# compbioproj-cdna-to-genome-map-align/gmap-2024

Measured on AMD Instinct MI355X. Metric: aligned cDNA reads/sec (2 kb, GRCh38) at 1/2/4/8 MI355X; DP HBM GB/s vs peak, higher is better.
Workload: dtype int32

## Files before the change

### gmap-2024_amd/csrc/oi_kernel.hip

```cpp
#include <cstdlib>

#include "dp_device.h"

namespace gmapdp {

constexpr int kOiK = 8;

#ifdef GMAPDP_OI_TIMING
__device__ unsigned long long g_oi_marks[2][16];
__device__ unsigned int g_oi_wave[3][16384];
#define OI_MARK(k)                                                 \
  do {                                                             \
    if (threadIdx.x == 0) {                                        \
      atomicAdd(&g_oi_marks[0][k], (unsigned long long)wall_clock64()); \
      atomicAdd(&g_oi_marks[1][k], 1ull);                          \
    }                                                              \
  } while (0)
#else
#define OI_MARK(k) \
  do {             \
  } while (0)
#endif
constexpr int kOiWords = 65536 / 32;

// ... 342 lines not shown
      c_mk = ((uint64_t)(uint32_t)__builtin_amdgcn_readlane((int)(mk >> 32), 63) << 32) |
             (uint32_t)__builtin_amdgcn_readlane((int)(uint32_t)mk, 63);
      c_key = KT::readlane(key_r, 63);
    }
  }
#pragma unroll
  for (int off = 32; off >= 1; off >>= 1) {
    const int om = __shfl_xor(bm, off, 64);
    const uint64_t ok = __shfl_xor(bkey, off, 64);
    const int oe = __shfl_xor(be, off, 64);
    if (om > bm || (om == bm && ok < bkey)) {
      bm = om;
      bkey = ok;
      be = oe;
    }
  }
  const int M = max(bm, 0);
  __threadfence_block();
  if (ngood == 0 && M > 0) {
    if (lane == 0) grec[0] = make_int4(-1, be, M, (int)(uint32_t)bkey);
    ngood = 1;
  }
  __threadfence_block();
  for (int g = lane; g < ngood; g += 64) {
    const int4 r = grec[g];
    const uint32_t di = (uint32_t)r.w;
    const int eb = r.y, bn = r.z;
    const uint32_t qreach = r.x >= 0 ? KT::q(S[r.x], cum, nq) : 0u;
    gkey[g] = ((uint64_t)qreach << 32) | di;
    grec[g] = make_int4(di >= (uint32_t)qlen ? (int)(di - (uint32_t)qlen) : (int)((uint32_t)qlen - di),
                        (int)KT::q(S[eb - bn], cum, nq), (int)KT::q(S[eb], cum, nq), bn + 1);
  }
  __threadfence_block();
  if (ngood > gcap) ngood = -1;
  for (int g = lane; g < ngood; g += 64) {
    const uint64_t k = gkey[g];
    int rank = 0;
    for (int h = 0; h < ngood; h++) rank += gkey[h] < k ? 1 : 0;
    reinterpret_cast<int4*>(good)[rank] = grec[g];
  }
  maxn_out = M;
  return ngood;
}

constexpr int kOimSlots = 1024;
__device__ __forceinline__ uint32_t oim_slot(uint32_t di) { return (di * 2654435761u) >> 22; }

template <typename KT, bool kSlots>
__device__ bool oi_mappings_sorted(int lane, int qlen, int nq, int E, uint32_t maxdiag, uint32_t chrinit,
                                   int lookback, int suffn, const int32_t* __restrict__ npq,
                                   const int32_t* __restrict__ mpq, const int* __restrict__ cum,
                                   const uint32_t* __restrict__ table_all, uint64_t* __restrict__ pool,
                                   unsigned long long base, uint32_t* hist,
                                   int* evq, int32_t* __restrict__ good, int gcap, int& ngood_out, int& maxn_out,
                                   uint32_t* slots = nullptr) {
  OI_MARK(9);
  if (base == ~0ull) return false;
  using K = typename KT::K;
  K* evA = reinterpret_cast<K*>(pool + base);
  K* evB = evA + E;
  int4* grec = reinterpret_cast<int4*>(pool + base + 2 * (size_t)E);
  const OiDigits D = oi_digits(maxdiag);
  const uint32_t need = (uint32_t)suffn + 1u;
  bool filtered = kSlots && E < 65536;
  if (filtered) {
    for (int i = lane; i < kOimSlots / 2; i += 64) slots[i] = 0u;
    oi_wave_sync();
    oi_for_events<KT>(lane, qlen, nq, chrinit, npq, mpq, cum, table_all, evq, [&](int, bool v, uint32_t di, K) {
      if (v) {
        const uint32_t h = oim_slot(di);
        atomicAdd(&slots[h >> 1], 1u << (16 * (h & 1)));
      }
    });
    oi_wave_sync();
  }
  for (;;) {
    for (int i = lane; i < kOiHist; i += 64) hist[i] = 0u;
    oi_wave_sync();
    int C = 0;
    oi_for_events<KT>(lane, qlen, nq, chrinit, npq, mpq, cum, table_all, evq,
                      [&](int, bool v, uint32_t di, K key) {
                        bool c = v;
                        if (filtered) {
                          const uint32_t h = oim_slot(di);
                          c = v && ((slots[h >> 1] >> (16 * (h & 1))) & 0xFFFFu) >= need;
                        }
                        const uint64_t cm = ballot(c);
                        if (c) evA[C + lanes_below(cm, lane)] = key;
                        oi_hist_add(lane, c, di, D, hist);
                        C += __popcll(cm);
                      });
    __threadfence_block();
    oi_wave_sync();
    OI_MARK(5);
    const K* S = oi_radix<KT>(lane, evA, evB, C, D, hist);
    OI_MARK(6);
    uint64_t* gkey = sizeof(K) == 8 ? reinterpret_cast<uint64_t*>(S == evA ? evB : evA) : pool + base + E;
    int maxn = 0;
    const int ngood = oi_sweep<KT>(lane, S, C, qlen, nq, lookback, suffn, cum, grec, gkey, good, gcap, maxn);
    if (filtered && ngood != -1 && (ngood == 0 || maxn < suffn)) {
      filtered = false;
      continue;
    }
    ngood_out = ngood;
    maxn_out = maxn;
    return true;
  }
}

template <typename CT>
__device__ __forceinline__ void count_inc(CT* cnt, int u) {
  if constexpr (sizeof(CT) == 4) {
    atomicAdd(reinterpret_cast<uint32_t*>(cnt) + u, 1u);
  } else {
    atomicAdd(reinterpret_cast<uint32_t*>(cnt) + (u >> 1), 1u << (16 * (u & 1)));
  }
}

__device__ void oi_report_overflow(const DevOligoProblem& P, int tid, int nthreads, int qlen, int32_t* npq,
                                   int32_t* mpq, gmapdp_oligo_result* results, unsigned char* poolslot) {
  for (int i = tid; i < qlen; i += nthreads) {
    npq[i] = 0;
    mpq[i] = -1;
  }
  if (tid == 0) {
    gmapdp_oligo_result res;
    res.totalpositions = 0;
    res.maxnconsecutive = 0;
    res.oned_matrix_p = -1;
    res.ndiagonals = 0;
    res.table_offset = P.table_offset;
    res.diag_offset = P.diag_offset;
    results[P.index] = res;
    *reinterpret_cast<unsigned long long*>(poolslot) = ~0ull;
  }
}

constexpr int kOiWaves = 2;
#ifdef GMAPDP_OI_STAGE
constexpr bool kOiStage = true;
#else
constexpr bool kOiStage = false;
#endif

#define OI_PASS_ARGS                                                                                          \
  const DevOligoProblem *__restrict__ probs, const uint32_t *__restrict__ blocks, const char *__restrict__ quc_all, \
      unsigned char *__restrict__ scratch, gmapdp_oligo_result *__restrict__ results,                             \
      int32_t *__restrict__ npos_out, int32_t *__restrict__ map_out, uint32_t *__restrict__ table_all,            \
      unsigned long long *__restrict__ pool_counter, unsigned long long pool_cap, int32_t *__restrict__ nhits_out
template <typename CT>
__device__ __forceinline__ void oi_pass(OI_PASS_ARGS) {
  extern __shared__ __attribute__((aligned(16))) unsigned char smem[];
  __shared__ int nh_wave[kOiWaves];
  const int tid = threadIdx.x, lane = tid & 63;
  const int wave = __builtin_amdgcn_readfirstlane(tid >> 6);
  const DevOligoProblem P = probs[blockIdx.x];
  uint32_t* bitmap = reinterpret_cast<uint32_t*>(smem);
  uint16_t* wrank = reinterpret_cast<uint16_t*>(smem + 4 * kOiWords);
  CT* cnt = reinterpret_cast<CT*>(smem + 6 * kOiWords);
  CT* offs = cnt + P.umax;
  const char* quc = quc_all + P.qoff;
  const int qlen = P.querylength;
  OI_MARK(0);
#ifdef GMAPDP_OI_TIMING
  const unsigned long long oi_t0 = wall_clock64();
#endif
  const int nq = qlen - kOiK + 1;

  for (int w = tid; w < kOiWords; w += 64 * kOiWaves) bitmap[w] = 0u;
  __syncthreads();
  int32_t* npq = npos_out + P.qoff;
  int32_t* mpq = map_out + P.qoff;
  for (int sb = 4 * 64 * wave; sb < qlen; sb += 4 * 64 * kOiWaves) {
    int ch[5];
#pragma unroll
    for (int r = 0; r < 5; r++) {
      const int i = sb + 64 * r + lane;
      ch[r] = i < qlen ? nt_code(quc[i]) : -1;
    }
#pragma unroll
    for (int r = 0; r < 4; r++) {
      const int i = sb + 64 * r + lane;
      uint32_t m = 0;
      bool ok = i < nq;
#pragma unroll
      for (int j = 0; j < kOiK; j++) {
        const int src = (lane + j) & 63;
        const int a = __shfl(ch[r], src, 64), b = __shfl(ch[r + 1], src, 64);
        const int cj = lane + j < 64 ? a : b;
        ok = ok && cj >= 0;
        m = (m << 2) | ((uint32_t)cj & 3u);
      }
      if (i < qlen) {
        mpq[i] = ok ? (int)m : -1;
        npq[i] = 0;
      }
      if (ok) atomicOr(&bitmap[m >> 5], 1u << (m & 31));
    }
  }
  __syncthreads();
  int run = 0;
  for (int base = 0; base < kOiWords; base += 64) {
    const int c = __popc(bitmap[base + lane]);
    const int incl = wave_scan_add(lane, c);
    if (wave == 0) wrank[base + lane] = (uint16_t)(run + incl - c);
    run += __builtin_amdgcn_readlane(incl, 63);
  }
  const int U = run;
  OI_MARK(1);
  unsigned char* base_s = scratch + P.scratch_offset;
  const ScratchOi so = scratch_oi(qlen, P.chrend > P.chrstart ? P.chrend - P.chrstart : 0);
  if (U > P.umax) {
    oi_report_overflow(P, tid, 64 * kOiWaves, qlen, npq, mpq, results, base_s + so.poolbase);
    return;
  }
  for (int u = tid; u < U; u += 64 * kOiWaves) cnt[u] = 0;
  __syncthreads();

  const uint64_t left = (uint64_t)P.chroffset + P.chrstart;
  uint64_t lpl = (uint64_t)P.chroffset + P.chrend + (P.plusp ? 0 : 1);
  lpl = lpl < (uint64_t)kOiK ? 0 : lpl - kOiK;
  const uint64_t npos = lpl > left ? lpl - left + 1 : 0;
  uint2* hitlist = reinterpret_cast<uint2*>(base_s + so.hits);
  uint32_t* hitlist32 = reinterpret_cast<uint32_t*>(base_s + so.hits);
  const bool compact = npos <= (1ull << 18);
  int nhits = 0;
  if (npos > 0) {
    const uint64_t hlo0 = left >> 4, hhi0 = lpl >> 4;
    const uint64_t nsteps = (hhi0 - hlo0) / 64 + 1, half = (nsteps + 1) / 2;
    const uint64_t hlo = hlo0 + (wave ? 64 * half : 0);
    const uint64_t hhi = wave ? hhi0 : (hlo0 + 64 * half - 1 < hhi0 ? hlo0 + 64 * half - 1 : hhi0);
    constexpr int kOiAhead = 4;
    uint32_t pw0[kOiAhead], pw1[kOiAhead];
#pragma unroll
    for (int a = 0; a < kOiAhead; a++) {
      const uint64_t hh = hlo + 64 * a + lane;
      pw0[a] = hh <= hhi ? half_word(blocks, hh) : 0u;
      pw1[a] = hh <= hhi ? half_word(blocks, hh + 1) : 0u;
    }
    auto step = [&](uint64_t hb, uint64_t v) {
      const uint64_t h = hb + lane;
      uint64_t vv;
      if (P.plusp) {
        vv = ((v >> 2) & 0x3333333333333333ull) | ((v & 0x3333333333333333ull) << 2);
        vv = ((vv >> 4) & 0x0F0F0F0F0F0F0F0Full) | ((vv & 0x0F0F0F0F0F0F0F0Full) << 4);
        vv = __builtin_bswap64(vv);
      } else {
        vv = ~v;
      }
      auto oligo_at = [&](int j) -> uint32_t {
        return (uint32_t)(vv >> (P.plusp ? 2 * (24 - j) : 2 * j)) & 0xFFFFu;
      };
      uint32_t vmask = 0;
      if (h <= hhi) {
        const uint64_t p0 = 16 * h;
        const int jlo = left > p0 ? (int)(left - p0) : 0;
        const int jhi = lpl < p0 + 15 ? (int)(lpl - p0) : 15;
        if (jlo <= jhi) vmask = (0xFFFFu >> (15 - jhi)) & (0xFFFFu << jlo);
      }
      uint32_t hm = 0;
#pragma unroll
      for (int j = 0; j < 16; j++) {
        const uint32_t m = oligo_at(j);
        hm |= ((bitmap[m >> 5] >> (m & 31)) & 1u) << j;
      }
      hm &= vmask;
      const int c = __popc(hm);
      const int incl = wave_scan_add(lane, c);
      int o = nhits + incl - c;
      for (uint32_t r = hm; r; r &= r - 1) {
        const int j = __ffs(r) - 1;
        const uint32_t m = oligo_at(j);
        bool in;
        const int id = oligo_id(bitmap, wrank, m, in);
        count_inc(cnt, id);
        if ((uint32_t)o < P.hit_cap) {
          const uint32_t at = wave ? P.hit_cap - 1 - (uint32_t)o : (uint32_t)o;
          const uint32_t k = (uint32_t)(16 * h + j - left);
          if (compact) hitlist32[at] = (k << 14) | (uint32_t)id;
          else hitlist[at] = make_uint2(k, (uint32_t)id);
        }
        o++;
      }
      nhits += __builtin_amdgcn_readlane(incl, 63);
    };
    for (uint64_t hb0 = hlo; hlo <= hhi && hb0 <= hhi; hb0 += 64 * kOiAhead) {
#pragma unroll
      for (int a = 0; a < kOiAhead; a++) {
        const uint64_t hb = hb0 + 64 * a;
        if (hb > hhi) break;
        const uint64_t v = (uint64_t)pw0[a] | ((uint64_t)pw1[a] << 32);
        const uint64_t hh = hb + 64 * kOiAhead + lane;
        pw0[a] = hh <= hhi ? half_word(blocks, hh) : 0u;
        pw1[a] = hh <= hhi ? half_word(blocks, hh + 1) : 0u;
        step(hb, v);
      }
    }
  }
  if (lane == 0) nh_wave[wave] = nhits;
  __syncthreads();
  const int n0 = nh_wave[0], n1 = nh_wave[1];
  nhits = n0 + n1;
  if (nhits_out && tid == 0) nhits_out[P.index] = nhits;
  __shared__ uint32_t tot_s;
  if (wave == 0) {
    uint32_t tot = 0;
    for (int base = 0; base < U; base += 64) {
      const int u = base + lane;
      const uint32_t c = u < U ? ((uint32_t)cnt[u] & 255u) : 0u;
      const uint32_t incl = (uint32_t)wave_scan_add(lane, (int)c);
      if (u < U) {
        offs[u] = (CT)(tot + incl - c);
        cnt[u] = (CT)c;
      }
      tot += (uint32_t)__builtin_amdgcn_readlane((int)incl, 63);
    }
    if (lane == 0) tot_s = tot;
  }
  for (int i = tid; i < nq; i += 64 * kOiWaves) {
    const int m = mpq[i];
    if (m >= 0) {
      bool in;
      mpq[i] = oligo_id(bitmap, wrank, (uint32_t)m, in);
    }
  }
  __syncthreads();
  const uint32_t tot = tot_s;
  OI_MARK(2);
  if ((uint32_t)nhits > P.hit_cap || tot > P.table_cap || (sizeof(CT) == 2 && nhits > 65535)) {
    oi_report_overflow(P, tid, 64 * kOiWaves, qlen, npq, mpq, results, base_s + so.poolbase);
    return;
  }

  uint32_t* table = table_all + P.table_offset;
  uint32_t* slotarr = hitlist32 + P.hit_cap;
  const uint32_t chrpos0 = P.plusp ? P.chrstart : (P.chrhigh - P.chroffset) - P.chrend;
  const int idbits = U > 1 ? 32 - __clz(U - 1) : 1;
  __threadfence_block();
  for (int c = 0; wave == 0 && c < nhits; c += 64) {
    const int sl = c + lane;
    int id = -1;
    uint32_t k = 0, at = 0;
    if (sl < nhits) {
      const int a = P.plusp ? nhits - 1 - sl : sl;
      at = a < n0 ? (uint32_t)a : P.hit_cap - 1 - (uint32_t)(a - n0);
      if (compact) {
        const uint32_t e = hitlist32[at];
        k = e >> 14;
        id = (int)(e & 0x3FFFu);
      } else {
        const uint2 hv = hitlist[at];
        k = hv.x;
        id = (int)hv.y;
      }
    }
    const uint64_t hits = ballot(id >= 0);
    uint64_t eq = hits;
    for (int b = 0; b < idbits; b++) {
      const uint64_t m = ballot((id >> b) & 1);
      eq &= ((id >> b) & 1) ? m : ~m;
    }
    if (id >= 0) {
      const int rank = lanes_below(eq, lane);
      const int same = __popcll(eq);
      const int r0 = (int)cnt[id];
      const uint32_t slot = (uint32_t)offs[id] + (uint32_t)(r0 - rank - 1);
      if (kOiStage && compact)
        slotarr[at] = r0 - rank > 0 ? slot : 0xFFFFFFFFu;
      else if (r0 - rank > 0)
        table[slot] = chrpos0 + (P.plusp ? k : (uint32_t)(npos - 1) - k);
      if (rank == 0) cnt[id] = (CT)max(r0 - same, 0);
    }
  }
  __threadfence_block();
  __syncthreads();
  if (kOiStage && compact) {
    uint32_t* stage = reinterpret_cast<uint32_t*>(smem);
    constexpr uint32_t kStage = 6 * kOiWords / 4;
    for (uint32_t b0 = 0; b0 < tot; b0 += kStage) {
      for (int a = tid; a < nhits; a += 64 * kOiWaves) {
        const uint32_t at = a < n0 ? (uint32_t)a : P.hit_cap - 1 - (uint32_t)(a - n0);
        const uint32_t sd = slotarr[at] - b0;
        if (sd < kStage) {
          const uint32_t k = hitlist32[at] >> 14;
          stage[sd] = chrpos0 + (P.plusp ? k : (uint32_t)(npos - 1) - k);
        }
      }
      __syncthreads();
      const uint32_t nb = min(kStage, tot - b0);
      for (uint32_t j = tid; j < nb; j += 64 * kOiWaves) table[b0 + j] = stage[j];
      __syncthreads();
    }
  }
  OI_MARK(3);
  for (int u = tid; u < U; u += 64 * kOiWaves)
    cnt[u] = (CT)((u + 1 < U ? (uint32_t)offs[u + 1] : tot) - (uint32_t)offs[u]);
  __threadfence_block();
  __syncthreads();
  if (wave) return;

  gmapdp_oligo_result res;
  res.totalpositions = 0;
  res.maxnconsecutive = 0;
  res.oned_matrix_p = 0;
  res.ndiagonals = 0;
  res.table_offset = P.table_offset;
  res.diag_offset = P.diag_offset;
  __threadfence_block();
  int* cum = reinterpret_cast<int*>(base_s);
  int totalpositions = 0, cumrun = 0;
  for (int sb = 0; sb < nq; sb += 4 * 64) {
    int mm[4];
#pragma unroll
    for (int r = 0; r < 4; r++) {
      const int i = sb + 64 * r + lane;
      mm[r] = i < nq ? mpq[i] : -1;
    }
#pragma unroll
    for (int r = 0; r < 4; r++) {
      const int i = sb + 64 * r + lane;
      const int m = mm[r];
      int nh = -1;
      if (i < nq) {
        int mo = -1;
        if (m >= 0) {
          const int u = m;
          nh = (int)cnt[u];
          npq[i] = nh;
          if (nh > 0) mo = (int32_t)(uint32_t)offs[u];
        }
        mpq[i] = mo;
      }
      const int incl = wave_scan_add(lane, nh == 0 ? 1 : 0);
      if (i < nq) cum[i] = cumrun + incl;
      cumrun += __builtin_amdgcn_readlane(incl, 63);
      totalpositions += __builtin_amdgcn_readlane(wave_scan_add(lane, nh > 0 ? nh : 0), 63);
    }
  }
  __threadfence_block();
  res.totalpositions = totalpositions;
  if (lane == 0) {
    results[P.index] = res;
    unsigned long long b = ~0ull;
    if (P.chrend > P.chrstart) {
      const unsigned long long need = 3ull * (unsigned long long)totalpositions;
      b = atomicAdd(pool_counter, need);
      if (b + need > pool_cap) b = ~0ull;
    }
    *reinterpret_cast<unsigned long long*>(base_s + so.poolbase) = b;
  }
  OI_MARK(4);
#ifdef GMAPDP_OI_TIMING
  if (lane == 0 && P.index < 16384) g_oi_wave[0][P.index] = (unsigned int)(wall_clock64() - oi_t0);
#endif
}

__device__ bool oi_mappings_walk(int lane, const DevOligoProblem& P, unsigned char* __restrict__ scratch, int qlen,
                                 int nq, const int32_t* __restrict__ npq, const int32_t* __restrict__ mpq,
                                 const int* __restrict__ cum, const uint32_t* __restrict__ table, uint32_t chrinit,
                                 int diag_lookback, int suffn, int32_t* __restrict__ good, int& ngood_out,
                                 int& maxn_out) {
  if (P.fallback_offset < 0) return false;
  const ScratchOiFb fb = scratch_oi_fb(qlen, P.chrend - P.chrstart);
  unsigned char* initp = scratch + P.fallback_offset + fb.initp;
  OiState* st = reinterpret_cast<OiState*>(scratch + P.fallback_offset + fb.states);
  for (size_t b = 16 * (size_t)lane; b < fb.states - fb.initp; b += 16 * 64)
    *reinterpret_cast<uint4*>(initp + b) = make_uint4(0u, 0u, 0u, 0u);
  __threadfence_block();
  int best = -1;
  int ngood = 0, maxn = 0;
  for (int cb = 0; cb < nq; cb += 64) {
    const int qi = cb + lane;
    int c_nh = 0, c_mo = 0, c_cum = 0;
    uint32_t c_h0 = 0;
    if (qi < nq) {
      c_nh = npq[qi];
      c_mo = mpq[qi];
      c_cum = cum[qi];
      if (c_nh > 0) c_h0 = table[c_mo];
    }
    const int cend = min(64, nq - cb);
    for (int j = 0; j < cend; j++) {
      const int nh = __builtin_amdgcn_readlane(c_nh, j);
      if (nh <= 0) continue;
      const int q = cb + j;
      const int mo = __builtin_amdgcn_readlane(c_mo, j);
      const int cq = __builtin_amdgcn_readlane(c_cum, j);
      const uint32_t h0 = (uint32_t)__builtin_amdgcn_readlane((int)c_h0, j);
      for (int base = 0; base < nh; base += 64) {
        const int h = base + lane;
        int reached = 0, nb = 0;
        uint32_t diagi = 0;
        if (h < nh) {
          diagi = (h == 0 ? h0 : table[mo + h]) + (uint32_t)(qlen - q) - chrinit;
          const unsigned char ini = initp[diagi];
          OiState s = st[diagi];
          if (!ini) {
            initp[diagi] = 1;
            s.querypos = -diag_lookback;
            s.best_n = s.n = s.cstart = s.best_start = s.best_end = 0;
          }
          if (s.querypos < 0) {
            s.n = 0;
            s.cstart = q;
          } else if (q - s.querypos >= diag_lookback + cq - cum[s.querypos]) {
            s.n = 0;
            s.cstart = q;
          } else if (++s.n > s.best_n) {
            s.best_start = s.cstart;
            s.best_end = q;
            s.best_n = s.n;
            reached = (s.best_n == suffn);
            nb = s.best_n;
          }
          s.querypos = q;
          st[diagi] = s;
        }
        const uint64_t rm = ballot(reached);
        if (reached && ngood + lanes_below(rm, lane) < (int)min(P.diag_cap, 0x7fffffffu))
          good[4 * (ngood + lanes_below(rm, lane))] = (int32_t)diagi;
        ngood += __popcll(rm);
        int mx = nb;
#pragma unroll
        for (int off = 32; off >= 1; off >>= 1) mx = max(mx, __shfl_xor(mx, off, 64));
        if (mx > maxn) {
          const int l = __ffsll((long long)ballot(nb == mx)) - 1;
          best = __builtin_amdgcn_readlane((int)diagi, l);
          maxn = mx;
        }
      }
    }
  }
  if (ngood == 0 && maxn > 0) {
    if (lane == 0 && P.diag_cap > 0) good[0] = best;
    ngood = 1;
  }
  __threadfence_block();
  if ((uint32_t)ngood > P.diag_cap) ngood = -1;
  for (int g = lane; g < ngood; g += 64) {
    const int di = good[4 * g];
    const OiState s = st[di];
    good[4 * g + 0] = di >= qlen ? di - qlen : qlen - di;
    good[4 * g + 1] = s.best_start;
    good[4 * g + 2] = s.best_end;
    good[4 * g + 3] = s.best_n + 1;
  }
  ngood_out = ngood;
  maxn_out = maxn;
  return true;
}

template <bool kSlots>
__device__ void oi_mappings_global(int lane, const DevOligoProblem& P, unsigned char* __restrict__ scratch, int qlen,
                                   int nq, int E, const int32_t* __restrict__ npq, const int32_t* __restrict__ mpq,
                                   const int* __restrict__ cum, const uint32_t* __restrict__ table,
                                   uint64_t* __restrict__ pool, unsigned long long pbase, uint32_t* hist, int* evq,
                                   int32_t* __restrict__ good, gmapdp_oligo_result* __restrict__ results,
                                   uint32_t* slots = nullptr) {
  const int diag_lookback = P.minor ? 60 : 120, suffn = P.minor ? 10 : 20;
  const uint32_t chrinit = P.plusp ? P.chrstart : (P.chrhigh - P.chroffset) - P.chrend;
  int ngood = 0, maxn = 0;
  const uint32_t maxdiag = (uint32_t)qlen + (P.chrend - P.chrstart);
  const int gcap = (int)min(P.diag_cap, 0x7fffffffu);
  const bool sorted =
      maxdiag < (1u << 20) - 1 && nq <= 4096
          ? oi_mappings_sorted<OiKeyT32, kSlots>(lane, qlen, nq, E, maxdiag, chrinit, diag_lookback, suffn, npq, mpq, cum,
                                         table, pool, pbase, hist, evq, good, gcap, ngood, maxn, slots)
      : nq < 65536
          ? oi_mappings_sorted<OiKeyQT, kSlots>(lane, qlen, nq, E, maxdiag, chrinit, diag_lookback, suffn, npq, mpq, cum,
                                        table, pool, pbase, hist, evq, good, gcap, ngood, maxn, slots)
          : oi_mappings_sorted<OiKeyQ, kSlots>(lane, qlen, nq, E, maxdiag, chrinit, diag_lookback, suffn, npq, mpq, cum,
                                       table, pool, pbase, hist, evq, good, gcap, ngood, maxn, slots);
  if (!sorted && !oi_mappings_walk(lane, P, scratch, qlen, nq, npq, mpq, cum, table, chrinit, diag_lookback, suffn,
                                   good, ngood, maxn))
    ngood = -1;
  if (lane == 0) {
    results[P.index].maxnconsecutive = ngood < 0 ? 0 : maxn;
    results[P.index].oned_matrix_p = ngood < 0 ? -1 : 1;
    results[P.index].ndiagonals = max(ngood, 0);
  }
}

template <typename CT>
__global__ __launch_bounds__(64 * kOiWaves) void oi_kernel(OI_PASS_ARGS) {
  oi_pass<CT>(probs, blocks, quc_all, scratch, results, npos_out, map_out, table_all, pool_counter, pool_cap,
              nhits_out);
}
template <typename CT>
__global__ __launch_bounds__(64 * kOiWaves) void oi_size_kernel(OI_PASS_ARGS) {
  oi_pass<CT>(probs, blocks, quc_all, scratch, results, npos_out, map_out, table_all, pool_counter, pool_cap,
              nhits_out);
}

#define OI_MAP_ARGS                                                                                           \
  const DevOligoProblem *__restrict__ probs, unsigned char *__restrict__ scratch,                                 \
      gmapdp_oligo_result *__restrict__ results, const int32_t *__restrict__ npos_out,                            \
      const int32_t *__restrict__ map_out, const uint32_t *__restrict__ table_all, int32_t *__restrict__ diag_all, \
      uint64_t *__restrict__ pool
__device__ __forceinline__ void oi_map_pass(OI_MAP_ARGS) {
  __shared__ uint32_t hist[kOiHist];
  __shared__ int evq[3 * 256];
  __shared__ uint32_t slots[kOimSlots / 2];
  const int lane = threadIdx.x;
  const DevOligoProblem P = probs[blockIdx.x];
  if (P.chrend <= P.chrstart) return;
  if (results[P.index].oned_matrix_p < 0) return;
  OI_MARK(8);
#ifdef GMAPDP_OI_TIMING
  const unsigned long long om_t0 = wall_clock64();
#endif
  const int qlen = P.querylength;
  const int nq = qlen - kOiK + 1;
  unsigned char* base_s = scratch + P.scratch_offset;
  const ScratchOi so = scratch_oi(qlen, P.chrend - P.chrstart);
  const int totalpositions = results[P.index].totalpositions;
  oi_mappings_global<true>(lane, P, scratch, qlen, nq, totalpositions, npos_out + P.qoff, map_out + P.qoff,
                     reinterpret_cast<const int*>(base_s), table_all + P.table_offset, pool,
                     *reinterpret_cast<const unsigned long long*>(base_s + so.poolbase), hist, evq,
                     diag_all + 4 * P.diag_offset, results, slots);
  OI_MARK(7);
#ifdef GMAPDP_OI_TIMING
  if (lane == 0 && P.index < 16384) {
    g_oi_wave[1][P.index] = (unsigned int)(wall_clock64() - om_t0);
    g_oi_wave[2][P.index] = (unsigned int)totalpositions;
  }
#endif
}

__global__ __launch_bounds__(64) void oi_map_kernel(OI_MAP_ARGS) {
  oi_map_pass(probs, scratch, results, npos_out, map_out, table_all, diag_all, pool);
}
__global__ __launch_bounds__(64) void oi_size_map_kernel(OI_MAP_ARGS) {
  oi_map_pass(probs, scratch, results, npos_out, map_out, table_all, diag_all, pool);
}


template <typename F>
__device__ __forceinline__ void oi_query_oligos(int lane, const char* __restrict__ quc, int qlen, int nq, int sb,
                                                F&& f) {
  int ch[5];
#pragma unroll
  for (int r = 0; r < 5; r++) {
    const int i = sb + 64 * r + lane;
    ch[r] = i < qlen ? nt_code(quc[i]) : -1;
  }
#pragma unroll
  for (int r = 0; r < 4; r++) {
    const int i = sb + 64 * r + lane;
    uint32_t m = 0;
    bool ok = i < nq;
#pragma unroll
    for (int j = 0; j < kOiK; j++) {
      const int src = (lane + j) & 63;
      const int a = __shfl(ch[r], src, 64), b = __shfl(ch[r + 1], src, 64);
      const int cj = lane + j < 64 ? a : b;
      ok = ok && cj >= 0;
      m = (m << 2) | ((uint32_t)cj & 3u);
    }
    f(i, ok, m);
  }
}

struct OiWindow {
  uint64_t left, lpl, npos;
  bool compact;
};
__device__ __forceinline__ OiWindow oi_window(const DevOligoProblem& P) {
  OiWindow w;
  w.left = (uint64_t)P.chroffset + P.chrstart;
  uint64_t lpl = (uint64_t)P.chroffset + P.chrend + (P.plusp ? 0 : 1);
  w.lpl = lpl < (uint64_t)kOiK ? 0 : lpl - kOiK;
  w.npos = w.lpl > w.left ? w.lpl - w.left + 1 : 0;
  w.compact = w.npos <= (1ull << 18);
  return w;
}

__global__ __launch_bounds__(64 * kOiWaves) void oi_scan_kernel(
    const DevOligoProblem* __restrict__ probs, const uint32_t* __restrict__ blocks, const char* __restrict__ quc_all,
    unsigned char* __restrict__ scratch, int32_t* __restrict__ npos_out, int32_t* __restrict__ map_out) {
  __shared__ uint32_t bitmap[kOiWords];
  __shared__ uint16_t wrank[kOiWords];
  __shared__ int nh_wave[kOiWaves];
  const int tid = threadIdx.x, lane = tid & 63;
  const int wave = __builtin_amdgcn_readfirstlane(tid >> 6);
  const DevOligoProblem P = probs[blockIdx.x];
  const char* quc = quc_all + P.qoff;
  const int qlen = P.querylength;
  const int nq = qlen - kOiK + 1;
  OI_MARK(10);
  for (int w = tid; w < kOiWords; w += 64 * kOiWaves) bitmap[w] = 0u;
  __syncthreads();
  for (int sb = 4 * 64 * wave; sb < qlen; sb += 4 * 64 * kOiWaves)
    oi_query_oligos(lane, quc, qlen, nq, sb, [&](int, bool ok, uint32_t m) {
      if (ok) atomicOr(&bitmap[m >> 5], 1u << (m & 31));
    });
  __syncthreads();
  int run = 0;
  for (int base = 0; base < kOiWords; base += 64) {
    const int c = __popc(bitmap[base + lane]);
    const int incl = wave_scan_add(lane, c);
    if (wave == 0) wrank[base + lane] = (uint16_t)(run + incl - c);
    run += __builtin_amdgcn_readlane(incl, 63);
  }
  const int U = run;
  __syncthreads();
  int32_t* npq = npos_out + P.qoff;
  int32_t* mpq = map_out + P.qoff;
  for (int sb = 4 * 64 * wave; sb < qlen; sb += 4 * 64 * kOiWaves)
    oi_query_oligos(lane, quc, qlen, nq, sb, [&](int i, bool ok, uint32_t m) {
      if (i < qlen) {
        bool in;
        mpq[i] = ok ? oligo_id(bitmap, wrank, m, in) : -1;
        npq[i] = 0;
      }
    });

  const OiWindow W = oi_window(P);
  const uint64_t left = W.left, lpl = W.lpl;
  unsigned char* base_s = scratch + P.scratch_offset;
  const ScratchOi so = scratch_oi(qlen, P.chrend > P.chrstart ? P.chrend - P.chrstart : 0);
  uint32_t* hl32 = reinterpret_cast<uint32_t*>(base_s + so.hits);
  uint2* hl64 = reinterpret_cast<uint2*>(base_s + so.hits);
  int nhits = 0;
  if (W.npos > 0) {
    const uint64_t hlo0 = left >> 4, hhi0 = lpl >> 4;
    const uint64_t nsteps = (hhi0 - hlo0) / 64 + 1, half = (nsteps + 1) / 2;
    const uint64_t hlo = hlo0 + (wave ? 64 * half : 0);
    const uint64_t hhi = wave ? hhi0 : (hlo0 + 64 * half - 1 < hhi0 ? hlo0 + 64 * half - 1 : hhi0);
    constexpr int kOiAhead = 4;
    uint32_t pw0[kOiAhead], pw1[kOiAhead];
#pragma unroll
    for (int a = 0; a < kOiAhead; a++) {
      const uint64_t hh = hlo + 64 * a + lane;
      pw0[a] = hh <= hhi ? half_word(blocks, hh) : 0u;
      pw1[a] = hh <= hhi ? half_word(blocks, hh + 1) : 0u;
    }
    auto step = [&](uint64_t hb, uint64_t v) {
      const uint64_t h = hb + lane;
      uint64_t vv;
      if (P.plusp) {
        vv = ((v >> 2) & 0x3333333333333333ull) | ((v & 0x3333333333333333ull) << 2);
        vv = ((vv >> 4) & 0x0F0F0F0F0F0F0F0Full) | ((vv & 0x0F0F0F0F0F0F0F0Full) << 4);
        vv = __builtin_bswap64(vv);
// ... 462 lines not shown
```

Measured before the change: 347,000.

## Fuse offset scan with per-query mapping pass and software-pipeline hit scatter loads

Merges the per-unique-oligo prefix scan, the oligo_id remapping loop and the final per-query cum/npq pass into a single wave-0 loop over queries. Offsets are assigned on first occurrence using ballot-based duplicate detection and a visited bit in cnt. The hit-scatter loop now prefetches the next batch of hitlist entries into registers before processing the current one. The per-unique recount pass is dropped. This removes two shared-memory passes and a block-wide remap loop, but the work is serialized onto one wave, adds extra ballots per query, and table order now follows first query occurrence.

```diff
diff --git a/gmap-2024_amd/csrc/oi_kernel.hip b/gmap-2024_amd/csrc/oi_kernel.hip
--- a/gmap-2024_amd/csrc/oi_kernel.hip
+++ b/gmap-2024_amd/csrc/oi_kernel.hip
@@ -668,27 +668,66 @@
   const int n0 = nh_wave[0], n1 = nh_wave[1];
   nhits = n0 + n1;
   if (nhits_out && tid == 0) nhits_out[P.index] = nhits;
+  for (int u = tid; u < U; u += 64 * kOiWaves) cnt[u] = (CT)((uint32_t)cnt[u] & 255u);
+  __syncthreads();
   __shared__ uint32_t tot_s;
+  const int idbits = U > 1 ? 32 - __clz(U - 1) : 1;
+  int* cum = reinterpret_cast<int*>(base_s);
+  int totalpositions = 0;
   if (wave == 0) {
     uint32_t tot = 0;
-    for (int base = 0; base < U; base += 64) {
-      const int u = base + lane;
-      const uint32_t c = u < U ? ((uint32_t)cnt[u] & 255u) : 0u;
-      const uint32_t incl = (uint32_t)wave_scan_add(lane, (int)c);
-      if (u < U) {
-        offs[u] = (CT)(tot + incl - c);
-        cnt[u] = (CT)c;
-      }
-      tot += (uint32_t)__builtin_amdgcn_readlane((int)incl, 63);
+    int cumrun = 0;
+    for (int sb = 0; sb < nq; sb += 4 * 64) {
+      int mm[4];
+#pragma unroll
+      for (int r = 0; r < 4; r++) {
+        const int i = sb + 64 * r + lane;
+        mm[r] = i < nq ? mpq[i] : -1;
+      }
+#pragma unroll
+      for (int r = 0; r < 4; r++) {
+        if (sb + 64 * r >= nq) break;
+        const int i = sb + 64 * r + lane;
+        int id = -1;
+        uint32_t cv = 0;
+        if (mm[r] >= 0) {
+          bool in;
+          id = oligo_id(bitmap, wrank, (uint32_t)mm[r], in);
+          cv = (uint32_t)cnt[id];
+        }
+        const bool cand = id >= 0 && (cv >> 8) == 0u;
+        uint64_t eq = ballot(cand);
+        for (int b = 0; b < idbits; b++) {
+          const uint64_t m = ballot((id >> b) & 1);
+          eq &= ((id >> b) & 1) ? m : ~m;
+        }
+        const bool first = cand && lanes_below(eq, lane) == 0;
+        const uint32_t kept = cv & 255u;
+        const uint32_t c = first ? kept : 0u;
+        const uint32_t incl = (uint32_t)wave_scan_add(lane, (int)c);
+        if (first) {
+          offs[id] = (CT)(tot + incl - c);
+          cnt[id] = (CT)(cv | 0x100u);
+        }
+        tot += (uint32_t)__builtin_amdgcn_readlane((int)incl, 63);
+        oi_wave_sync();
+        int nh = -1;
+        if (i < nq) {
+          int mo = -1;
+          if (id >= 0) {
+            nh = (int)kept;
+            npq[i] = nh;
+            if (nh > 0) mo = (int32_t)(uint32_t)offs[id];
+          }
+          mpq[i] = mo;
+        }
+        const int cincl = wave_scan_add(lane, nh == 0 ? 1 : 0);
+        if (i < nq) cum[i] = cumrun + cincl;
+        cumrun += __builtin_amdgcn_readlane(cincl, 63);
+        totalpositions += __builtin_amdgcn_readlane(wave_scan_add(lane, nh > 0 ? nh : 0), 63);
+      }
     }
     if (lane == 0) tot_s = tot;
-  }
-  for (int i = tid; i < nq; i += 64 * kOiWaves) {
-    const int m = mpq[i];
-    if (m >= 0) {
-      bool in;
-      mpq[i] = oligo_id(bitmap, wrank, (uint32_t)m, in);
-    }
   }
   __syncthreads();
   const uint32_t tot = tot_s;
@@ -701,41 +740,62 @@
   uint32_t* table = table_all + P.table_offset;
   uint32_t* slotarr = hitlist32 + P.hit_cap;
   const uint32_t chrpos0 = P.plusp ? P.chrstart : (P.chrhigh - P.chroffset) - P.chrend;
-  const int idbits = U > 1 ? 32 - __clz(U - 1) : 1;
   __threadfence_block();
-  for (int c = 0; wave == 0 && c < nhits; c += 64) {
-    const int sl = c + lane;
-    int id = -1;
-    uint32_t k = 0, at = 0;
-    if (sl < nhits) {
-      const int a = P.plusp ? nhits - 1 - sl : sl;
-      at = a < n0 ? (uint32_t)a : P.hit_cap - 1 - (uint32_t)(a - n0);
-      if (compact) {
-        const uint32_t e = hitlist32[at];
-        k = e >> 14;
-        id = (int)(e & 0x3FFFu);
-      } else {
-        const uint2 hv = hitlist[at];
-        k = hv.x;
-        id = (int)hv.y;
-      }
-    }
-    const uint64_t hits = ballot(id >= 0);
-    uint64_t eq = hits;
-    for (int b = 0; b < idbits; b++) {
-      const uint64_t m = ballot((id >> b) & 1);
-      eq &= ((id >> b) & 1) ? m : ~m;
-    }
-    if (id >= 0) {
-      const int rank = lanes_below(eq, lane);
-      const int same = __popcll(eq);
-      const int r0 = (int)cnt[id];
-      const uint32_t slot = (uint32_t)offs[id] + (uint32_t)(r0 - rank - 1);
-      if (kOiStage && compact)
-        slotarr[at] = r0 - rank > 0 ? slot : 0xFFFFFFFFu;
-      else if (r0 - rank > 0)
-        table[slot] = chrpos0 + (P.plusp ? k : (uint32_t)(npos - 1) - k);
-      if (rank == 0) cnt[id] = (CT)max(r0 - same, 0);
+  constexpr int kP2 = 4;
+  uint32_t at_n[kP2];
+  uint2 hv_n[kP2];
+  auto load_hits = [&](int c0) {
+#pragma unroll
+    for (int r = 0; r < kP2; r++) {
+      const int sl = c0 + 64 * r + lane;
+      at_n[r] = 0;
+      hv_n[r] = make_uint2(0u, 0xFFFFFFFFu);
+      if (wave == 0 && sl < nhits) {
+        const int a = P.plusp ? nhits - 1 - sl : sl;
+        const uint32_t at = a < n0 ? (uint32_t)a : P.hit_cap - 1 - (uint32_t)(a - n0);
+        at_n[r] = at;
+        if (compact) {
+          const uint32_t e = hitlist32[at];
+          hv_n[r] = make_uint2(e >> 14, e & 0x3FFFu);
+        } else {
+          hv_n[r] = hitlist[at];
+        }
+      }
+    }
+  };
+  load_hits(0);
+  for (int c0 = 0; wave == 0 && c0 < nhits; c0 += 64 * kP2) {
+    uint32_t at_c[kP2];
+    uint2 hv_c[kP2];
+#pragma unroll
+    for (int r = 0; r < kP2; r++) {
+      at_c[r] = at_n[r];
+      hv_c[r] = hv_n[r];
+    }
+    load_hits(c0 + 64 * kP2);
+#pragma unroll
+    for (int r = 0; r < kP2; r++) {
+      if (c0 + 64 * r >= nhits) break;
+      const uint32_t at = at_c[r], k = hv_c[r].x;
+      const int id = (int)hv_c[r].y;
+      const uint64_t hits = ballot(id >= 0);
+      uint64_t eq = hits;
+      for (int b = 0; b < idbits; b++) {
+        const uint64_t m = ballot((id >> b) & 1);
+        eq &= ((id >> b) & 1) ? m : ~m;
+      }
+      if (id >= 0) {
+        const int rank = lanes_below(eq, lane);
+        const int same = __popcll(eq);
+        const uint32_t cv = (uint32_t)cnt[id];
+        const int r0 = (int)(cv & 255u);
+        const uint32_t slot = (uint32_t)offs[id] + (uint32_t)(r0 - rank - 1);
+        if (kOiStage && compact)
+          slotarr[at] = r0 - rank > 0 ? slot : 0xFFFFFFFFu;
+        else if (r0 - rank > 0)
+          table[slot] = chrpos0 + (P.plusp ? k : (uint32_t)(npos - 1) - k);
+        if (rank == 0) cnt[id] = (CT)(cv - (uint32_t)min(same, r0));
+      }
     }
   }
   __threadfence_block();
@@ -759,52 +819,18 @@
     }
   }
   OI_MARK(3);
-  for (int u = tid; u < U; u += 64 * kOiWaves)
-    cnt[u] = (CT)((u + 1 < U ? (uint32_t)offs[u + 1] : tot) - (uint32_t)offs[u]);
   __threadfence_block();
   __syncthreads();
   if (wave) return;
 
   gmapdp_oligo_result res;
-  res.totalpositions = 0;
+  res.totalpositions = totalpositions;
   res.maxnconsecutive = 0;
   res.oned_matrix_p = 0;
   res.ndiagonals = 0;
   res.table_offset = P.table_offset;
   res.diag_offset = P.diag_offset;
   __threadfence_block();
-  int* cum = reinterpret_cast<int*>(base_s);
-  int totalpositions = 0, cumrun = 0;
-  for (int sb = 0; sb < nq; sb += 4 * 64) {
-    int mm[4];
-#pragma unroll
-    for (int r = 0; r < 4; r++) {
-      const int i = sb + 64 * r + lane;
-      mm[r] = i < nq ? mpq[i] : -1;
-    }
-#pragma unroll
-    for (int r = 0; r < 4; r++) {
-      const int i = sb + 64 * r + lane;
-      const int m = mm[r];
-      int nh = -1;
-      if (i < nq) {
-        int mo = -1;
-        if (m >= 0) {
-          const int u = m;
-          nh = (int)cnt[u];
-          npq[i] = nh;
-          if (nh > 0) mo = (int32_t)(uint32_t)offs[u];
-        }
-        mpq[i] = mo;
-      }
-      const int incl = wave_scan_add(lane, nh == 0 ? 1 : 0);
-      if (i < nq) cum[i] = cumrun + incl;
-      cumrun += __builtin_amdgcn_readlane(incl, 63);
-      totalpositions += __builtin_amdgcn_readlane(wave_scan_add(lane, nh > 0 ? nh : 0), 63);
-    }
-  }
-  __threadfence_block();
-  res.totalpositions = totalpositions;
   if (lane == 0) {
     results[P.index] = res;
     unsigned long long b = ~0ull;
```

Result: faster. 351,200, median of 6 (+1.2%).
